# iamwinter/UMPR

Hardware: AMD Instinct MI355X
Metric: training samples/sec (higher is better)
Workload: dtype f32

## Files before the change

### include/umpr_hip.h

```cpp
#ifndef UMPR_HIP_H
#define UMPR_HIP_H
#include <stddef.h>
#include <stdint.h>

#ifdef __cplusplus
extern "C" {
#endif

const char* umpr_version(void);
const char* umpr_last_error(void);
int umpr_device_info(int dev, char* name, int name_len, int* compute_units, size_t* hbm_bytes);

int umpr_gemm_f32(const float* A, long lda, int transA, const float* B, long ldb, int transB, float* C, long ldc,
                  int M, int N, int K, const float* bias, int bias_mode, int act, int accumulate, float alpha,
                  float* ws, size_t ws_bytes, void* stream);

int umpr_set_gemm_bf16(int on);

int umpr_set_conv_inference(int on);

int umpr_set_conv_pool_follows(int on);

long umpr_debug_wino_fix_count(void);

int umpr_debug_conv3x3_plan(int pass, int N, int Cin, int Cout, int H, int W, int inference, size_t* ws_bytes, size_t* v_bytes);

int umpr_debug_wino_pool_fold(const float* y, const float* g_pooled, const float* w, const float* x, float* unpooled, float* dx,
                              float* dw, float* db, int N, int Cin, int Cout, int H, int W, int f4, int fold, float* ws,
                              size_t ws_bytes, void* stream);

size_t umpr_embed_gru_bidir_ws_bytes(int N, int L, int E);
int umpr_embed_gru_bidir_fwd(const int64_t* ids, const float* emb, int E,
                             const float* w_ih_f, const float* w_hh_f, const float* b_ih_f, const float* b_hh_f,
                             const float* w_ih_r, const float* w_hh_r, const float* b_ih_r, const float* b_hh_r,
                             const int32_t* lengths, const int32_t* order, const int32_t* dst_row, int N, int L,
                             float* out, float* saved, float* ws, size_t ws_bytes, void* stream);
int umpr_embed_gru_bidir_bwd(const int64_t* ids, const float* emb, int E,
                             const float* w_hh_f, const float* w_hh_r,
                             const int32_t* lengths, const int32_t* order, const int32_t* dst_row, int N, int L,
                             const float* dout, const float* out, const float* saved,
                             float* dw_ih_f, float* dw_hh_f, float* db_ih_f, float* db_hh_f,
                             float* dw_ih_r, float* dw_hh_r, float* db_ih_r, float* db_hh_r,
                             float* ws, size_t ws_bytes, void* stream);

int umpr_embed_gru_bidir_bwd_acc(const int64_t* ids, const float* emb, int E,
                                 const float* w_hh_f, const float* w_hh_r,
                                 const int32_t* lengths, const int32_t* order, const int32_t* dst_row, int N, int L,
                                 const float* dout, const float* out, const float* saved,
                                 float* dw_ih_f, float* dw_hh_f, float* db_ih_f, float* db_hh_f,
                                 float* dw_ih_r, float* dw_hh_r, float* db_ih_r, float* db_hh_r,
                                 int accumulate, float* ws, size_t ws_bytes, void* stream);

int umpr_embed_gru_bidir_bwd_dx(const int64_t* ids, const float* emb, int E,
                                const float* w_hh_f, const float* w_hh_r,
                                const int32_t* lengths, const int32_t* order, const int32_t* dst_row, int N, int L,
                                const float* dout, const float* out, const float* saved,
                                float* dw_ih_f, float* dw_hh_f, float* db_ih_f, float* db_hh_f,
                                float* dw_ih_r, float* dw_hh_r, float* db_ih_r, float* db_hh_r,
                                int accumulate, const float* w_ih_f, const float* w_ih_r, float* dx, int dx_accumulate,
                                float* ws, size_t ws_bytes, void* stream);

int umpr_embed_grad_chunk(void);
size_t umpr_embed_grad_ws_bytes(long T, int E);
int umpr_embed_grad(const int64_t* const* ids, const float* const* dx, const long* counts, int n_src, int E, long vocab,
                    const int32_t* sorted_pos, float* d_emb, void* ws, size_t ws_bytes, void* stream);

size_t umpr_embed_grad_rows_ws_bytes(long T, int E);
int umpr_embed_grad_rows(const int64_t* const* ids, const float* const* dx, const long* counts, int n_src, int E, long vocab,
                         const int32_t* sorted_pos, int64_t* row_id, float* row_grad, void* ws, size_t ws_bytes, void* stream);
int umpr_sparse_adam_rows(float* p, float* m, float* v, long vocab, int E, const int64_t* row_id, const float* row_grad, long T,
                          double lr, double beta1, double beta2, double eps, long step, double grad_scale,
                          const float* clip_state , void* stream);

size_t umpr_coattention_fwd_ws_bytes(int B, int SL);
int umpr_coattention_fwd(const float* Gu, const float* Gi, const float* M, int B, int SL, float* T, float* soft_u,
                         float* soft_i, float* atte_u, long ld_u, float* atte_i, long ld_i, float* colmax,
// ... 271 lines not shown
```

### umpr_amd/_lib.py

```python
from __future__ import annotations

import ctypes
import os
import threading

import torch

_HERE = os.path.dirname(os.path.abspath(__file__))
LIB_PATH = os.path.join(_HERE, "libumpr_hip.so")

_T = {"p": ctypes.c_void_p, "i": ctypes.c_int, "l": ctypes.c_long, "z": ctypes.c_size_t, "f": ctypes.c_float,
      "d": ctypes.c_double, "u": ctypes.c_uint64}

SIGNATURES = {
    "umpr_version": ("", "s"),
    "umpr_last_error": ("", "s"),
    "umpr_device_info": ("ipipp", "i"),
    "umpr_gemm_f32": ("pliplipliiipiiifpzp", "i"),
    "umpr_embed_gru_bidir_ws_bytes": ("iii", "z"),
    "umpr_embed_gru_bidir_fwd": ("ppipppppppppppiipppzp", "i"),
    "umpr_embed_gru_bidir_bwd": ("ppipppppiippppppppppppzp", "i"),
    "umpr_embed_gru_bidir_bwd_acc": ("ppipppppiipppppppppppipzp", "i"),
    "umpr_embed_gru_bidir_bwd_dx": ("ppipppppiipppppppppppipppipzp", "i"),
    "umpr_embed_grad_chunk": ("", "i"),
# ... 57 lines not shown
    "umpr_vgg16_bf16_act_bytes": ("i", "z"),
    "umpr_vgg16_bf16_fwd_ws_bytes": ("i", "z"),
    "umpr_vgg16_bf16_bwd_ws_bytes": ("i", "z"),
    "umpr_vgg16_bf16_features_fwd": ("ppipppzp", "i"),
    "umpr_vgg16_bf16_features_bwd": ("ppippppzp", "i"),
    "umpr_vgg16_cls_arena_bytes": ("i", "z"),
    "umpr_vgg16_classifier_fwd_compact": ("piiiuppppzp", "i"),
    "umpr_vgg16_classifier_bwd_compact": ("piippppppzp", "i"),
    "umpr_vgg16_classifier_fwd_compact_bf16": ("piiiuppppzp", "i"),
    "umpr_vgg16_classifier_bwd_compact_bf16": ("piippppppzp", "i"),
    "umpr_concat_ids": ("pplpp", "i"),
    "umpr_review_net_arena_bytes": ("iii", "z"),
    "umpr_review_net_ws_bytes": ("iiii", "z"),
    "umpr_review_net_fwd": ("ppipppiiiiiipppzp", "i"),
    "umpr_review_net_fwd_masked": ("ppipppiiiiiipppzpp", "i"),
    "umpr_review_net_bwd": ("ppipppiiiippppzp", "i"),
    "umpr_review_net_bwd_dx": ("ppipppiiiipppppzp", "i"),
    "umpr_review_net_fwd_ex": ("ppippppiiiiiipppzpp", "i"),
    "umpr_review_net_bwd_ex": ("ppippppiiiipppppzp", "i"),
    "umpr_control_net_arena_bytes": ("iiiiiii", "z"),
    "umpr_control_net_ws_bytes": ("iiiiiiiii", "z"),
    "umpr_control_net_fwd": ("pppipppppiiiiiiiifiippppppzp", "i"),
    "umpr_control_net_bwd": ("pppipppppiiiiiiiiipppppppzp", "i"),
    "umpr_control_net_bwd_dx": ("pppipppppiiiiiiiiipppppppppzp", "i"),
    "umpr_control_net_fwd_ex": ("pppipppppppiiiiiiiifiippppppzppp", "i"),
    "umpr_control_net_bwd_ex": ("pppipppppppiiiiiiiiipppppppppzp", "i"),
    "umpr_head_fwd": ("pppppppppppppfiiipppppppp", "i"),
    "umpr_head_bwd": ("pppppppppppfiiippppppppppppppppppppp", "i"),
    "umpr_photo_resize_u8": ("pzpiiipp", "i"),
    "umpr_photo_store_slot_bytes": ("ii", "z"),
    "umpr_photo_fetch_u8": ("pzpppiiiplpp", "i"),
    "umpr_photo_fetch_augment_u8": ("pzppppiiiplplpppp", "i"),
    "umpr_feature_fetch_f32": ("pipppiiplpp", "i"),
    "umpr_review_collate": ("pplppppppplpiiiiilpppp", "i"),
    "umpr_review_collate_sampled": ("pplppppppplpiiiiil" "iuil" "pppp", "i"),
    "umpr_bce_head_fwd": ("plpppiipppzp", "i"),
    "umpr_bce_head_bwd": ("plpppppiiplpppzp", "i"),
    "umpr_adam_step": ("ppppldddddldp", "i"),
    "umpr_sq_err_accumulate": ("pplpp", "i"),
    "umpr_adam_step_dev": ("pppplddd" "pp", "i"),
    "umpr_grad_norm_ws_bytes": ("", "z"),
    "umpr_grad_norm": ("ppidfppzpp", "i"),
    "umpr_adam_step_clip": ("ppppldddddld" "pp", "i"),
    "umpr_adam_step_dev_clip": ("pppplddd" "ppp", "i"),
    "umpr_adam_step_groups": ("ppppldddddld" "pp" "ppp" "ii" "p", "i"),
    "umpr_grad_accumulate": ("pppiip", "i"),
    "umpr_ema_update": ("pppidip", "i"),
    "umpr_arena_swap": ("pppip", "i"),
    "umpr_debug_poison_lds": ("pp", "i"),
    "umpr_set_gemm_bf16": ("i", "i"),
    "umpr_set_conv_inference": ("i", "i"),
    "umpr_set_conv_pool_follows": ("i", "i"),
    "umpr_debug_wino_fix_count": ("", "l"),
    "umpr_debug_conv3x3_plan": ("iiiiiiipp", "i"),
    "umpr_debug_wino_pool_fold": ("pppppppp" "iiiiiii" "pzp", "i"),
    "umpr_profile_enable": ("i", "i"),
    "umpr_profile_reset": ("", "i"),
    "umpr_profile_read": ("ippp", "i"),
}


class UmprHipError(RuntimeError):
    pass


class _Tls(threading.local):
    gemm_b16 = False


TLS = _Tls()


class _Lib:
    def __init__(self):
        if not os.path.exists(LIB_PATH):
            raise UmprHipError(
                f"{LIB_PATH} not found: build it with `python -c 'import __graft_entry__ as g; g.build()'` "
                f"(or `make -C umpr_amd/csrc`).  There is no CPU fallback.")
        self.cdll = ctypes.CDLL(LIB_PATH)
        self.fn = {}
        for name, (args, ret) in SIGNATURES.items():
            f = getattr(self.cdll, name)
            f.argtypes = [_T[c] for c in args]
            f.restype = {"i": ctypes.c_int, "z": ctypes.c_size_t, "s": ctypes.c_char_p, "p": ctypes.c_void_p,
                         "l": ctypes.c_long}[ret]
            self.fn[name] = f

    def last_error(self) -> str:
        return self.fn["umpr_last_error"]().decode()

    def call(self, name, *args):
        conv = []
        for a in args:
            if isinstance(a, torch.Tensor):
                conv.append(a.data_ptr())
            elif a is None:
                conv.append(None)
            else:
                conv.append(a)
        if TLS.gemm_b16:
            self.fn["umpr_set_gemm_bf16"](1)
            try:
                rc = self.fn[name](*conv)
            finally:
                self.fn["umpr_set_gemm_bf16"](0)
        else:
# ... 37 lines not shown
```

### umpr_amd/csrc/api.hip

```cpp
#include <math.h>
#include <stdarg.h>
#include <stdlib.h>

#include <vector>

#include "../../include/umpr_hip.h"
#include "umpr_common.h"
#include "umpr_internal.h"

static thread_local char g_err[512] = "";
void umpr_set_error(const char* fmt, ...) {
  va_list ap;
  va_start(ap, fmt);
  vsnprintf(g_err, sizeof(g_err), fmt, ap);
  va_end(ap);
}

namespace {
const bool g_fc_small = umpr_env_on("UMPR_FC_SMALL");
struct ProfRec { hipEvent_t e0, e1; int family; double work; };
bool g_prof_on = false;
std::vector<ProfRec> g_prof;
std::vector<ProfRec> g_prof_pool;
double g_prof_ms[UMPR_K_COUNT] = {0}, g_prof_work[UMPR_K_COUNT] = {0};
// ... 37 lines not shown
    for (int j = 0; j < kConvPerBlock[b]; ++j) {
      L.conv_cin[ci] = cin; L.conv_cout[ci] = kBlockCh[b]; L.conv_hw[ci] = hw; L.conv_block[ci] = b;
      L.conv_off[ci] = off;
      off += (size_t)n * kBlockCh[b] * hw * hw;
      cin = kBlockCh[b];
      ++ci;
    }
    hw /= 2;
    L.pool_off[b] = off;
    off += (size_t)n * kBlockCh[b] * hw * hw;
  }
  for (int j = 0; j < 2; ++j) { L.fc_off[j] = off; off += (size_t)n * 4096; }
  for (int j = 0; j < 2; ++j) { L.drop_off[j] = off; off += (size_t)n * 4096; }
  for (int i = 0; i < 13; ++i) {
    L.v_floats[i] = umpr_conv3x3_plan(CONV_FWD, n, L.conv_cin[i], L.conv_cout[i], L.conv_hw[i], L.conv_hw[i], false).v_floats;
    L.v_off[i] = off;
    off += L.v_floats[i];
  }
  L.total = off;
  return L;
}
}

extern "C" {

const char* umpr_version(void) { return "umpr_hip 0.1 (gfx950)"; }
const char* umpr_last_error(void) { return g_err; }

int umpr_device_info(int dev, char* name, int name_len, int* compute_units, size_t* hbm_bytes) {
  hipDeviceProp_t prop;
  if (hipGetDeviceProperties(&prop, dev) != hipSuccess) { umpr_set_error("device_info: no device %d", dev); return -1; }
  if (name && name_len > 0) { strncpy(name, prop.name, name_len - 1); name[name_len - 1] = 0; }
  if (compute_units) *compute_units = prop.multiProcessorCount;
  if (hbm_bytes) *hbm_bytes = prop.totalGlobalMem;
  return 0;
}

int umpr_gemm_f32(const float* A, long lda, int transA, const float* B, long ldb, int transB, float* C, long ldc,
                  int M, int N, int K, const float* bias, int bias_mode, int act, int accumulate, float alpha,
                  float* ws, size_t ws_bytes, void* stream) {
  UmprGemm g;
  g.A = A; g.lda = lda; g.transA = transA != 0; g.B = B; g.ldb = ldb; g.transB = transB != 0; g.C = C; g.ldc = ldc;
  g.M = M; g.N = N; g.K = K; g.bias = bias; g.bias_mode = bias_mode; g.act = act; g.accumulate = accumulate != 0;
  g.alpha = alpha; g.split_k = ws ? 0 : 1; g.ws = ws; g.ws_bytes = ws_bytes;
  return umpr_gemm(g, S(stream));
}

int umpr_set_gemm_bf16(int on) { umpr_gemm_set_b16(on != 0); return 0; }
static thread_local bool t_conv_inference = false, t_conv_pool_follows = false;
int umpr_set_conv_inference(int on) { t_conv_inference = on != 0; return 0; }
int umpr_set_conv_pool_follows(int on) { t_conv_pool_follows = on != 0; return 0; }
static ConvHints conv_hints() { ConvHints h; h.inference = t_conv_inference; h.pool_follows = t_conv_pool_follows; return h; }
long umpr_debug_wino_fix_count(void) { return umpr_wino_last_fix_count(); }
int umpr_debug_conv3x3_plan(int pass, int N, int Cin, int Cout, int H_, int W, int inference, size_t* ws_bytes, size_t* v_bytes) {
  UMPR_REQUIRE(pass >= CONV_FWD && pass <= CONV_WGRAD && N > 0 && Cin > 0 && Cout > 0 && H_ > 0 && W > 0, "conv3x3_plan: bad arguments");
  const ConvPlan p = umpr_conv3x3_plan(static_cast<ConvPass>(pass), N, Cin, Cout, H_, W, inference != 0);
  if (ws_bytes) *ws_bytes = p.ws_floats * sizeof(float);
  if (v_bytes) *v_bytes = p.v_floats * sizeof(float);
  return p.algo;
}
int umpr_debug_wino_pool_fold(const float* y, const float* g_pooled, const float* w, const float* x, float* unpooled, float* dx,
                              float* dw, float* db, int N, int Cin, int Cout, int H_, int W, int f4, int fold, float* ws,
                              size_t ws_bytes, void* stream) {
  UMPR_REQUIRE(N > 0 && Cin > 0 && Cout > 0 && H_ > 0 && W > 0 && (H_ % 2) == 0 && (W % 2) == 0 && y && g_pooled && ws,
               "debug_wino_pool_fold: bad arguments");
  UMPR_REQUIRE(fold || unpooled, "debug_wino_pool_fold: the un-folded run needs the buffer for the un-pooled gradient");
  UMPR_REQUIRE(!dx || (f4 && w), "debug_wino_pool_fold: the data gradient runs on the 4x4 tile and needs the weights");
  UMPR_REQUIRE(!dw || (x && (!f4 || ((H_ % 4) == 0 && (W % 4) == 0))), "debug_wino_pool_fold: the weight gradient on the 4x4 tile has no edge tiles");
  hipStream_t s = S(stream);
  ConvHints h;
  const float* g = g_pooled;
  if (fold) { h.pooled_dy = true; h.pool_y = y; }
  else {
    if (int rc = umpr_maxpool2_bwd_relu_impl(y, g_pooled, unpooled, (long)N * Cout, H_, W, s)) return rc;
    g = unpooled;
  }
  if (dx)
    if (int rc = umpr_wino_conv3x3(g, w, 1, nullptr, nullptr, dx, N, Cin, Cout, H_, W, 0, ws, ws_bytes / sizeof(float), true, h, s)) return rc;
  if (dw)
    if (int rc = umpr_wino_wgrad(g, x, dw, db, N, Cin, Cout, H_, W, 0, ws, ws_bytes / sizeof(float), f4 != 0, h, s)) return rc;
  return 0;
}

constexpr size_t kSlabs = 256;
namespace {
struct GruWs {
  float *gx, *wslab, *bslab;
  float* kslab; size_t kslab_bytes;
  float *stacked, *rows;
  float *wst, *bst;
  size_t bytes;
};
GruWs gru_ws(float* base, int N, int L, int pitch) {
  Carve c(base, sizeof(float));
  const size_t tiles = umpr_gru_tiles(N);
  GruWs w;
  w.gx = c.take<float>((size_t)N * L * 384); w.wslab = c.take<float>(tiles * 2 * G3 * H); w.bslab = c.take<float>(tiles * 2 * 2 * G3);
  w.wst = c.at<float>(c.off); w.bst = c.at<float>(c.off + (size_t)2 * G3 * pitch * sizeof(float));
  w.kslab_bytes = kSlabs * G3 * pitch * sizeof(float); w.kslab = c.take<float>(kSlabs * G3 * pitch);
  w.stacked = c.take<float>((size_t)2 * G3 * pitch); w.rows = c.take<float>((size_t)N * L * pitch); w.bytes = c.off;
  return w;
}
const bool g_emb_gather = umpr_env_on("UMPR_EMB_GATHER");
__global__ __launch_bounds__(256) void gather_rows_kernel(const int64_t* __restrict__ ids, const float* __restrict__ emb,
                                                          int E, int Ep, float* __restrict__ out, long rows) {
  const int lane = threadIdx.x & 63;
// ... 933 lines not shown
```

### umpr_amd/csrc/umpr_internal.h

```cpp
#pragma once
#include <hip/hip_runtime.h>
#include <stdint.h>

struct UmprGemm {
  const float* A = nullptr; long lda = 0; bool transA = false;
  const float* B = nullptr; long ldb = 0; bool transB = false;
  float* C = nullptr; long ldc = 0;
  int M = 0, N = 0, K = 0;
  const int64_t* gatherA = nullptr;
  const int64_t* gatherB = nullptr;
  const float* bias = nullptr; int bias_mode = 0;
  int act = 0; bool accumulate = false; float alpha = 1.0f;
  int split_k = 1;
  float* ws = nullptr; size_t ws_bytes = 0;
  int winA_L = 0, winA_D = 1, winA_pad = 0;
  int winB_L = 0, winB_D = 1, winB_pad = 0;
};
void umpr_gemm_set_b16(int on);
int umpr_gemm_b16();
int umpr_gemm(const UmprGemm& g, hipStream_t stream);
struct UmprB16Scope {
  int prev;
  explicit UmprB16Scope(int on) : prev(umpr_gemm_b16()) { if (on) umpr_gemm_set_b16(1); }
  ~UmprB16Scope() { umpr_gemm_set_b16(prev); }
// ... 25 lines not shown

int umpr_fill(float* p, long n, float v, hipStream_t s);
int umpr_multi_copy(const float* const* src, float* const* dst, const long* n, const int* accumulate, int nseg, hipStream_t s);
int umpr_multi_colsum_rows(const float* const* src, const int* rows, const long* cols, const long* row_stride, float* const* dst,
                           const int* accumulate, int nseg, hipStream_t s);
int umpr_copy_or_add(const float* src, float* dst, long n, int accumulate, hipStream_t s);

struct UmprHead {
  const float* rr;
  const float* c_u; const float* c_i; const float* pp; const float* pn;
  const float* vgg;
  const float* pos_v; const float* neg_v;
  const float* lw; const float* lb;
  const float* fw; const float* fb;
  const float* labels;
  float rate;
  int B, V, P, F;
  float* pred; float* loss;
  float* z;
  float* img_emb; float* pos_match; float* neg_match;
  float* posneg_emb;
  const float* d_loss;
  const float* d_pred;
  float* d_rr; float* d_cu; float* d_ci; float* d_pp; float* d_pn;
  float* d_vgg; float* d_pos_v; float* d_neg_v; float* d_lw; float* d_lb; float* d_fw; float* d_fb;
};
int umpr_head_launch(const UmprHead& p, int backward, hipStream_t s);

enum ConvPass { CONV_FWD = 0, CONV_DGRAD = 1, CONV_WGRAD = 2 };
enum ConvAlgo { CONV_GENERIC = 0 , CONV_C3 = 1 ,
                CONV_DIRECT = 2 , CONV_WINO2 = 3, CONV_WINO4 = 4 };
struct ConvHints {
  bool inference = false, pool_follows = false; float* v_slot = nullptr; size_t v_slot_floats = 0;
  bool pooled_dy = false; const float* pool_y = nullptr;
};
struct ConvPlan {
  ConvAlgo algo;
  ConvAlgo direct;
  bool edge;
  size_t ws_floats;
  size_t v_floats;
};
ConvPlan umpr_conv3x3_plan(ConvPass pass, int N, int Cin, int Cout, int H, int W, bool inference);
size_t umpr_conv3x3_pack_floats(int N, int Cin, int Cout, int H, int W);
bool umpr_conv3x3_pool_fold_ok(int N, int Cin, int Cout, int H, int W);
int umpr_conv3x3_run(const float* x, const float* w, int transposed, const float* bias, const float* mask, float* y,
                     int N, int Cin, int Cout, int H, int W, int relu, float* wpack, size_t wpack_floats,
                     const ConvHints& hints, hipStream_t s);
struct WinoConvGeom { int planes, MT, S; long T, Tpad; bool edge; size_t v_floats, U, V, M, count, tie, floats; };
WinoConvGeom umpr_wino_conv_geom(int N, int C, int M, int H, int W, bool f4);
struct WinoWgradGeom { long T, Tpad; int MT, CT, Mpad, Cpad, stages, splits, stages_per_split, planes, bnc; size_t Gy, V, P, BP, floats; };
WinoWgradGeom umpr_wino_wgrad_geom(int N, int Cin, int Cout, int H, int W, bool f4);
long umpr_wino_last_fix_count();
int umpr_wino_wgrad(const float* dy, const float* x, float* dw, float* db, int N, int Cin, int Cout, int H, int W,
                    int accumulate, float* ws, size_t ws_floats, bool f4, const ConvHints& hints, hipStream_t s);
int umpr_wino_conv3x3(const float* x, const float* w, int transposed, const float* bias, const float* mask, float* y,
                      int N, int Cin, int Cout, int H, int W, int relu, float* ws, size_t ws_floats, bool f4,
                      const ConvHints& hints, hipStream_t s);
int umpr_conv3x3_flip_transpose(const float* w, float* wt, int Cout, int Cin, hipStream_t s);
size_t umpr_conv3x3_wgrad_ws_bytes(int N, int Cin, int Cout, int H, int W);
int umpr_conv3x3_wgrad(const float* gz, const float* x, float* dw, float* db, int N, int Cin, int Cout, int H, int W,
                       int accumulate, float* ws, size_t ws_bytes, const ConvHints& hints, hipStream_t s);
int umpr_maxpool2_fwd_impl(const float* x, float* y, long planes, int H, int W, hipStream_t s);
int umpr_maxpool2_bwd_relu_impl(const float* x, const float* gy, float* gx, long planes, int H, int W, hipStream_t s);

int umpr_wgrad_reduce(const float* slab, const float* bslab, int splits, int Cout, int Cin, float* dw, float* db,
                      int accumulate, hipStream_t s);

struct UmprPF {
  int N, H, W, RW;
  long rows;
  long ptot;
  long lead, tail;
  long ps;
};
UmprPF umpr_pf(int N, int H, int W);
size_t umpr_pf_bytes(const UmprPF& g, int C);
size_t umpr_conv_bf16_pack_bytes(int Cin, int Cout);
int umpr_conv_bf16_run(const void* x, const float* w, int transposed, const float* bias, const void* mask, void* y,
                       const UmprPF& g, int Cin, int Cout, int relu, void* wpack, size_t wpack_bytes, hipStream_t s,
                       bool zero_guards = true);
int umpr_conv_bf16_pack_all(const float* const* w, const int* Cin, const int* Cout, const int* W, int n, int transposed,
                            void* wpack, const size_t* offsets, hipStream_t s);
int umpr_pf_zero_guards_multi(void* const* bases, const UmprPF* geos, const int* channels, int n, hipStream_t s);
size_t umpr_wgrad_bf16_ws_bytes(const UmprPF& g, int Cin, int Cout);
int umpr_wgrad_bf16_run(const void* dy, const void* x, float* dw, float* db, const UmprPF& g, int Cin, int Cout,
                        int accumulate, float* ws, size_t ws_bytes, hipStream_t s);
int umpr_conv1_bf16_fwd(const float* x, const float* w, const float* bias, void* y, const UmprPF& g, hipStream_t s,
                        bool zero_guards = true);
size_t umpr_conv1_bf16_wgrad_ws_bytes();
int umpr_conv1_bf16_wgrad(const void* dy, const float* x, float* dw, float* db, const UmprPF& g, int accumulate, float* ws,
                          size_t ws_bytes, hipStream_t s);
int umpr_nchw_to_cb8(const float* x, void* y, const UmprPF& g, int C, hipStream_t s);
int umpr_cb8_to_nchw(const void* x, float* y, const UmprPF& g, int C, hipStream_t s);
int umpr_maxpool2_bf16_fwd_run(const void* x, void* y, const UmprPF& gi, const UmprPF& go, int C, hipStream_t s,
                               bool zero_guards = true);
int umpr_maxpool2_bf16_bwd_run(const void* x, const void* gy, void* gx, const UmprPF& gi, const UmprPF& go, int C,
                               hipStream_t s);

int umpr_colsum_rows(const float* src, int rows, long cols, long row_stride, float* dst, int accumulate, hipStream_t s);
int umpr_gru_recurrent_fwd(const float* gx, const float* whh_f, const float* bhh_f, const float* whh_r,
                           const float* bhh_r, const int* lengths, const int* order, const int* dst_row, float* out,
                           float* saved, int N, int L, hipStream_t s);
int umpr_gru_tiles(int N);
int umpr_gru_bptt(const float* dout, const float* out, const float* saved, const float* whh_f, const float* whh_r,
                  const int* lengths, const int* order, const int* dst_row, float* dgx, float* dwhh_slab,
// ... 69 lines not shown
```

### umpr_amd/csrc/winograd.hip

```cpp
#include <type_traits>

#include "umpr_common.h"
#include "umpr_internal.h"

namespace {

constexpr int WK = 32;
constexpr int WBM = 128;
constexpr int WBN = 128;

__device__ __forceinline__ void pool_window_grad(const float2 a, const float2 b, const float gy, float2& ga, float2& gb) {
  int arg = 0;
  float m = a.x;
  if (a.y > m) { m = a.y; arg = 1; }
  if (b.x > m) { m = b.x; arg = 2; }
  if (b.y > m) { m = b.y; arg = 3; }
  const float g = m > 0.f ? gy : 0.f;
  ga = make_float2(arg == 0 ? g : 0.f, arg == 1 ? g : 0.f);
  gb = make_float2(arg == 2 ? g : 0.f, arg == 3 ? g : 0.f);
}
typedef float f32x4_t __attribute__((ext_vector_type(4)));
__device__ __forceinline__ float as_loaded(float v) { asm volatile("" : "+v"(v)); return v; }
__device__ __forceinline__ float4 as_loaded(const float4 v) {
  f32x4_t q = {v.x, v.y, v.z, v.w};
  asm volatile("" : "+v"(q));
  return make_float4(q.x, q.y, q.z, q.w);
}

__global__ void wino_weights_kernel(const float* __restrict__ w, float* __restrict__ U, int M, int C, int CinW,
                                    int transposed) {
  const int MT = (M + WBM - 1) / WBM, S = (C + WK - 1) / WK;
  const long total = (long)MT * WBM * S * WK;
  for (long i = blockIdx.x * (long)blockDim.x + threadIdx.x; i < total; i += (long)gridDim.x * blockDim.x) {
    const int ml = (int)(i % WBM);
    long r = i / WBM;
    const int k = (int)(r % WK); r /= WK;
    const int s = (int)(r % S);
    const int mt = (int)(r / S);
    const int m = mt * WBM + ml, c = s * WK + k;
    float g[9];
#pragma unroll
    for (int t = 0; t < 9; ++t) {
      float v = 0.f;
      if (m < M && c < C) v = transposed ? w[((long)c * CinW + m) * 9 + 8 - t] : w[((long)m * CinW + c) * 9 + t];
      g[t] = v;
    }
    float gg[4][3];
#pragma unroll
    for (int j = 0; j < 3; ++j) {
      gg[0][j] = g[j];
      gg[1][j] = 0.5f * (g[j] + g[3 + j] + g[6 + j]);
      gg[2][j] = 0.5f * (g[j] - g[3 + j] + g[6 + j]);
// ... 598 lines not shown
                                                         const unsigned int* __restrict__ list, const unsigned int* __restrict__ count,
                                                         unsigned cap, int C, int Mch, int H, int W, int relu) {
  const unsigned n_fix = min(*count, cap);
  const int lane = threadIdx.x & 63;
  const unsigned wave = blockIdx.x * 4 + (threadIdx.x >> 6), waves = gridDim.x * 4;
  const long HW = (long)H * W;
  for (unsigned i = wave; i < n_fix; i += waves) {
    const unsigned idx = list[i];
    const int xx = (int)(idx % W);
    unsigned r = idx / W;
    const int yy = (int)(r % H); r /= H;
    const int m = (int)(r % Mch);
    const int n = (int)(r / Mch);
    float acc = 0.f;
    for (int c = lane; c < C; c += 64) {
      const float* xp = x + ((long)n * C + c) * HW;
      const float* wp = w + ((long)m * C + c) * 9;
#pragma unroll
      for (int dy = 0; dy < 3; ++dy) {
        const int py = yy + dy - 1;
        if (py < 0 || py >= H) continue;
#pragma unroll
        for (int dx = 0; dx < 3; ++dx) {
          const int px = xx + dx - 1;
          if (px < 0 || px >= W) continue;
          acc = fmaf(xp[(long)py * W + px], wp[dy * 3 + dx], acc);
        }
      }
    }
#pragma unroll
    for (int o = 32; o > 0; o >>= 1) acc += __shfl_xor(acc, o, 64);
    if (lane == 0) {
      float v = acc + (bias ? bias[m] : 0.f);
      if (relu) v = fmaxf(v, 0.f);
      y[idx] = v;
    }
  }
}

static long wino_tpad(long T) { return (T + WBN - 1) / WBN * WBN; }

struct WinoGemmParams {
  const float* U;
  const float* V;
  float* Mx;
  int MT, S, C;
  long Tpad;
  long TT;
  int Mpad;
  int planes;
};

typedef __attribute__((address_space(3))) void* lds_ptr_t;
template <int FOLD>
__global__ __launch_bounds__(256, 2) void wino_gemm_dma_kernel(WinoGemmParams p) {
  constexpr int SK = WK;
  constexpr int LD = 128;
  constexpr int TM = 2, TN = 2;
  constexpr int KS = SK / 2;
  constexpr int NP = SK / 8;
  constexpr int SFLUSH = 1;
  typedef typename std::conditional<FOLD == 2, double, float>::type tot_t;
  __shared__ __attribute__((aligned(1024))) float As[2][SK * LD];
  __shared__ __attribute__((aligned(1024))) float Bs[2][SK * LD];
  const int tid = threadIdx.x, lane = tid & 63;
  const int wave = __builtin_amdgcn_readfirstlane(tid >> 6);
  const int wm = wave >> 1, wn = wave & 1;
  const int l31 = lane & 31, half = lane >> 5;
  const long TT = p.TT;
  const int xcd = blockIdx.x & 7;
  const long qq = blockIdx.x >> 3;
  const int mt = (int)(qq % p.MT);
  const long bt = (qq / p.MT) * 8 + xcd;
  if (bt >= p.planes * TT) return;
  const int xi = (int)(bt / TT);
  const long t0 = (bt % TT) * WBN;
  const float* Ub = p.U + (((long)xi * p.MT + mt) * p.S) * (WK * WBM);
  const float* Vb = p.V + (long)xi * (p.S * WK) * p.Tpad + t0;
  const float* ga = Ub + wave * (NP * 256) + lane * 4;
  const float* gb = Vb + (long)(wave * (2 * NP) + half) * p.Tpad + l31 * 4;
  const long bstep = 2 * p.Tpad;
  const unsigned lds_a = (unsigned)(size_t)(lds_ptr_t)(&As[0][0]) + (unsigned)wave * (NP * 1024u);
  const unsigned lds_b = (unsigned)(size_t)(lds_ptr_t)(&Bs[0][0]) + (unsigned)wave * (NP * 1024u);
  auto glds = [&](const float* src, unsigned dst) {
    unsigned keep;
    asm volatile("s_mov_b32 %0, m0\n\ts_mov_b32 m0, %2\n\ts_nop 0\n\tglobal_load_lds_dwordx4 %1, off\n\ts_mov_b32 m0, %0"
                 : "=&s"(keep) : "v"(src), "s"(dst) : "memory");
  };
  auto dma = [&](int q, int sn, int nbuf) {
    if (q < NP) glds(ga + (long)sn * (SK * WBM) + q * 256, lds_a + (unsigned)nbuf * (SK * LD * 4u) + (unsigned)q * 1024u);
    else glds(gb + (long)sn * SK * p.Tpad + (q - NP) * bstep, lds_b + (unsigned)nbuf * (SK * LD * 4u) + (unsigned)(q - NP) * 1024u);
  };
  auto dma_wait = [&]() { asm volatile("s_waitcnt vmcnt(0)" ::: "memory"); };

  f32x16 acc[TM][TN];
  tot_t tot[TM][TN][16];
#pragma unroll
  for (int i = 0; i < TM; ++i)
#pragma unroll
    for (int j = 0; j < TN; ++j)
#pragma unroll
      for (int r = 0; r < 16; ++r) { acc[i][j][r] = 0.f; tot[i][j][r] = (tot_t)0; }

  const int ns = p.S * (WK / SK);
#pragma unroll
  for (int q = 0; q < 2 * NP; ++q) dma(q, 0, 0);
  dma_wait();
  __syncthreads();
  for (int s0 = 0; s0 < ns; s0 += SFLUSH) {
#pragma unroll
    for (int i = 0; i < TM; ++i)
#pragma unroll
      for (int j = 0; j < TN; ++j)
#pragma unroll
        for (int r = 0; r < 16; ++r) acc[i][j][r] = 0.f;
    const int s1 = min(ns, s0 + SFLUSH);
    for (int s = s0; s < s1; ++s) {
      const int cur = s & 1;
      const int sn = min(s + 1, ns - 1);
      const float* as = As[cur] + half * LD + wm * 64 + l31;
      const float* bs = Bs[cur] + half * LD + wn * 64 + l31;
      float a[2][TM], b[2][TN];
#pragma unroll
      for (int i = 0; i < TM; ++i) a[0][i] = as[i * 32];
#pragma unroll
      for (int j = 0; j < TN; ++j) b[0][j] = bs[j * 32];
#pragma unroll
      for (int kk = 0; kk < KS; ++kk) {
        const int cb = kk & 1, nb = cb ^ 1;
        const int k1 = kk + 1;
#pragma unroll
        for (int m = 0; m < TM * TN; ++m) {
          const int i = m / TN, j = m % TN;
          acc[i][j] = mfma32(a[cb][i], b[cb][j], acc[i][j]);
          if (m == 0 && k1 < KS) {
#pragma unroll
            for (int ii = 0; ii < TM; ++ii) a[nb][ii] = as[2 * k1 * LD + ii * 32];
          }
          if (m == 1 && k1 < KS) {
#pragma unroll
            for (int jj = 0; jj < TN; ++jj) b[nb][jj] = bs[2 * k1 * LD + jj * 32];
          }
          if (m == 3 && kk < 2 * NP) dma(kk, sn, cur ^ 1);
          __builtin_amdgcn_sched_barrier(0);
        }
      }
      dma_wait();
      __syncthreads();
    }
#pragma unroll
    for (int i = 0; i < TM; ++i)
#pragma unroll
      for (int j = 0; j < TN; ++j)
#pragma unroll
        for (int r = 0; r < 16; ++r) tot[i][j][r] += (tot_t)acc[i][j][r];
  }
  float* Mb = p.Mx + ((long)xi * p.Mpad + mt * WBM) * p.Tpad + t0;
#pragma unroll
  for (int i = 0; i < TM; ++i)
#pragma unroll
    for (int j = 0; j < TN; ++j)
#pragma unroll
      for (int r = 0; r < 16; ++r)
        Mb[(long)(wm * 64 + i * 32 + mfma_row(r, lane)) * p.Tpad + wn * 64 + j * 32 + l31] = (float)tot[i][j][r];
}

inline int nblk(long n, int cap) {
  long b = (n + 255) / 256;
  if (b > cap) b = cap;
  return (int)(b < 1 ? 1 : b);
}

}

static thread_local const unsigned int* t_last_fix_count = nullptr;
long umpr_wino_last_fix_count() {
  if (!t_last_fix_count) return -1;
  unsigned int v = 0;
  if (hipDeviceSynchronize() != hipSuccess || hipMemcpy(&v, t_last_fix_count, sizeof(v), hipMemcpyDeviceToHost) != hipSuccess) return -2;
  return (long)v;
}

WinoConvGeom umpr_wino_conv_geom(int N, int C, int M, int H, int W, bool f4) {
  WinoConvGeom g;
  g.planes = f4 ? 36 : 16; g.edge = f4 && ((H % 4) != 0 || (W % 4) != 0);
  g.T = f4 ? (long)N * ((H + 3) / 4) * ((W + 3) / 4) : (long)N * (H / 2) * (W / 2);
  g.Tpad = wino_tpad(g.T); g.MT = (M + WBM - 1) / WBM; g.S = (C + WK - 1) / WK;
  g.v_floats = (size_t)g.planes * g.S * WK * g.Tpad;
  g.U = 0; g.V = (size_t)g.planes * g.MT * WBM * g.S * WK; g.M = g.V + g.v_floats;
  g.count = g.M + (size_t)g.planes * g.MT * WBM * g.Tpad; g.tie = g.count + 16;
  g.floats = g.count + 64 + (f4 ? g.Tpad : 0);
  return g;
}


int umpr_wino_conv3x3(const float* x, const float* w, int transposed, const float* bias, const float* mask, float* y,
                      int N, int Cin, int Cout, int H, int W, int relu, float* ws, size_t ws_floats, bool f4,
                      const ConvHints& hints, hipStream_t s) {
  const int M = transposed ? Cin : Cout;
  const int C = transposed ? Cout : Cin;
  const WinoConvGeom G = umpr_wino_conv_geom(N, C, M, H, W, f4);
  UMPR_REQUIRE(ws_floats >= G.floats, "winograd: workspace too small");
  UMPR_REQUIRE((H % 2) == 0 && (W % 2) == 0, "winograd: odd map %dx%d", H, W);
  const int planes = G.planes, MT = G.MT, S = G.S;
  const long T = G.T, Tpad = G.Tpad; const bool edge = G.edge;
  float *U = ws + G.U, *V = ws + G.V, *Mx = ws + G.M, *list_region = ws + G.V;
  if (hints.v_slot) {
    UMPR_REQUIRE(f4 && !edge && !transposed && hints.v_slot_floats == G.v_floats,
                 "winograd: the V slot does not fit this forward (%d -> %d at %dx%d)", Cin, Cout, H, W);
    V = hints.v_slot;
  }
  if (f4) wino4_weights_kernel<<<nblk((long)MT * WBM * S * WK, 2048), 256, 0, s>>>(w, U, M, C, Cin, transposed, wino4_consts());
  else wino_weights_kernel<<<nblk((long)MT * WBM * S * WK, 2048), 256, 0, s>>>(w, U, M, C, Cin, transposed);
  UMPR_LAUNCH_CHECK("wino_weights");
  const long TT = (T + WBN - 1) / WBN;
  static const int kappa = umpr_env_int("UMPR_WINO_FIX_KAPPA", 8);
  const bool fix = f4 && !transposed && !hints.inference && kappa > 0 && mask == nullptr;
  WinoFix fx{nullptr, nullptr, 0u, 0.f, nullptr};
  unsigned int* tie_bits = nullptr;
  if (fix) {
    fx.count = reinterpret_cast<unsigned int*>(ws + G.count);
    fx.list = reinterpret_cast<unsigned int*>(list_region);
    fx.cap = (unsigned)(G.v_floats < (size_t)0x7fffffff ? G.v_floats : (size_t)0x7fffffff);
    fx.kappa_eps = (float)kappa * 5.9604644775390625e-08f;
    UMPR_REQUIRE((long)N * M * H * W < 0xffffffffL, "winograd fix-up: output tensor too large for 32-bit element indices");
    if (hints.pool_follows) {
      tie_bits = reinterpret_cast<unsigned int*>(ws + G.tie);
      if (hipMemsetAsync(tie_bits - 1, 0, (size_t)(T + 1) * sizeof(unsigned int), s) != hipSuccess) { umpr_set_error("winograd fix-up: memset"); return -2; }
      UMPR_REQUIRE(((long)N * C * H * W) % 4 == 0 && (reinterpret_cast<uintptr_t>(x) & 15) == 0, "winograd fix-up: unaligned input");
      wino_absmax_kernel<<<nblk((long)N * C * H * W / 4, 1024), 256, 0, s>>>(x, (long)N * C * H * W / 4, tie_bits - 1);
      UMPR_LAUNCH_CHECK("wino_absmax");
      fx.tie_bits = tie_bits;
    }
  }
  if (hints.pooled_dy) {
    UMPR_REQUIRE(f4 && transposed && hints.pool_y && !fix, "winograd: the pooled source needs a data gradient on the 4x4 tile");
    if (edge) wino4_input_kernel<true, false, true><<<nblk((long)S * WK * TT * WBN, 16384), 256, 0, s>>>(x, V, N, C, S * WK, H, W, Tpad, TT * WBN, wino4_consts(), nullptr, nullptr, hints.pool_y);
    else wino4_input_kernel<false, false, true><<<nblk((long)S * WK * TT * WBN, 16384), 256, 0, s>>>(x, V, N, C, S * WK, H, W, Tpad, TT * WBN, wino4_consts(), nullptr, nullptr, hints.pool_y);
  } else if (f4 && edge) {
    if (tie_bits) wino4_input_kernel<true, true><<<nblk((long)S * WK * TT * WBN, 16384), 256, 0, s>>>(x, V, N, C, S * WK, H, W, Tpad, TT * WBN, wino4_consts(), fx.count, tie_bits);
    else wino4_input_kernel<true, false><<<nblk((long)S * WK * TT * WBN, 16384), 256, 0, s>>>(x, V, N, C, S * WK, H, W, Tpad, TT * WBN, wino4_consts(), fx.count, nullptr);
  } else if (f4) {
    if (tie_bits) wino4_input_kernel<false, true><<<nblk((long)S * WK * TT * WBN, 16384), 256, 0, s>>>(x, V, N, C, S * WK, H, W, Tpad, TT * WBN, wino4_consts(), fx.count, tie_bits);
    else wino4_input_kernel<false, false><<<nblk((long)S * WK * TT * WBN, 16384), 256, 0, s>>>(x, V, N, C, S * WK, H, W, Tpad, TT * WBN, wino4_consts(), fx.count, nullptr);
  }
  else if ((W / 2) % 2 == 0)
    wino_input_pair_kernel<<<nblk((long)S * WK * TT * WBN / 2, 16384), 256, 0, s>>>(x, V, N, C, S * WK, H, W, Tpad, TT * WBN);
  else
    wino_input_kernel<<<nblk((long)S * WK * TT * WBN, 16384), 256, 0, s>>>(x, V, N, C, S * WK, H, W, Tpad, TT * WBN);
  UMPR_LAUNCH_CHECK("wino_input");
  WinoGemmParams p{U, V, Mx, MT, S, C, Tpad, TT, MT * WBM, planes};
  const long groups = (planes * TT + 7) / 8 * 8;
  {
    UmprProfScope prof(UMPR_K_WINO_GEMM, 2.0 * planes * (double)M * C * T, s);
    static const int fold = umpr_env_int("UMPR_WINO_FOLD", 1);
    if (fold == 2) wino_gemm_dma_kernel<2><<<(unsigned)(groups * MT), 256, 0, s>>>(p);
    else wino_gemm_dma_kernel<1><<<(unsigned)(groups * MT), 256, 0, s>>>(p);
  }
  UMPR_LAUNCH_CHECK("wino_gemm");
  if (f4 && fix) {
    if (edge) wino4_output_kernel<true, true><<<nblk((long)M * T, 16384), 256, 0, s>>>(Mx, bias, mask, y, N, M, H, W, Tpad, MT * WBM, relu, wino4_consts(), fx);
    else wino4_output_kernel<false, true><<<nblk((long)M * T, 16384), 256, 0, s>>>(Mx, bias, mask, y, N, M, H, W, Tpad, MT * WBM, relu, wino4_consts(), fx);
    UMPR_LAUNCH_CHECK("wino_output");
    wino_fixup_kernel<<<128, 256, 0, s>>>(x, w, bias, y, fx.list, fx.count, fx.cap, C, M, H, W, relu);
    UMPR_LAUNCH_CHECK("wino_fixup");
    t_last_fix_count = fx.count;
    return 0;
  }
  if (f4 && edge)
    wino4_output_kernel<true, false><<<nblk((long)M * T, 16384), 256, 0, s>>>(Mx, bias, mask, y, N, M, H, W, Tpad, MT * WBM, relu, wino4_consts(), fx);
  else if (f4)
    wino4_output_kernel<false, false><<<nblk((long)M * T, 16384), 256, 0, s>>>(Mx, bias, mask, y, N, M, H, W, Tpad, MT * WBM, relu, wino4_consts(), fx);
  else if ((W / 2) % 2 == 0)
    wino_output_pair_kernel<<<nblk((long)M * T / 2, 16384), 256, 0, s>>>(Mx, bias, mask, y, N, M, H, W, Tpad, MT * WBM, relu);
  else
    wino_output_kernel<<<nblk((long)M * T, 16384), 256, 0, s>>>(Mx, bias, mask, y, N, M, H, W, Tpad, MT * WBM, relu);
  UMPR_LAUNCH_CHECK("wino_output");
  return 0;
}

namespace {

template <bool POOL>
__global__ void wino_dy_kernel(const float* __restrict__ dy, float* __restrict__ Gy, int N, int Mch, int H, int W,
                               long Tpad, long Tw, int Mpad, const float* __restrict__ pool_y) {
  const int TH = H / 2, TW = W / 2;
  const long T = (long)N * TH * TW;
  const long total = (long)Mch * Tw;
  const long per = (long)Mpad * Tpad;
  for (long i = blockIdx.x * (long)blockDim.x + threadIdx.x; i < total; i += (long)gridDim.x * blockDim.x) {
    const long t = i % Tw;
    const int m = (int)(i / Tw);
    float* dst = Gy + (long)m * Tpad + t;
    if (t >= T) {
#pragma unroll
      for (int a = 0; a < 16; ++a) dst[(long)a * per] = 0.f;
      continue;
    }
    const int tx = (int)(t % TW);
    const long r = t / TW;
    const int ty = (int)(r % TH), n = (int)(r / TH);
    const long o = (((long)n * Mch + m) * H + 2 * ty) * W + 2 * tx;
    float2 g0, g1;
    if (POOL) {
      pool_window_grad(*reinterpret_cast<const float2*>(pool_y + o), *reinterpret_cast<const float2*>(pool_y + o + W),
                       dy[((long)n * Mch + m) * TH * TW + (long)ty * TW + tx], g0, g1);
    } else {
      g0 = *reinterpret_cast<const float2*>(dy + o);
      g1 = *reinterpret_cast<const float2*>(dy + o + W);
    }
// ... 573 lines not shown
```

Measured before the change: 2184.

## Add 64-column Winograd GEMM tile variant chosen by a wave-quantization cost model

Templates the Winograd batched GEMM kernel on its column tile width, adding a 64-wide variant with smaller LDS footprint and three workgroups per CU. A host-side cost model compares rounds of workgroups across the device's CUs for both widths and picks 64 when the 128 grid would leave a partially filled final wave. This targets tail-wave underutilization on layers whose block count does not divide evenly across CUs, at the cost of less B-tile reuse per workgroup and a heuristic constant that may mispredict. A debug override and a query API are also exposed.

```diff
diff --git a/include/umpr_hip.h b/include/umpr_hip.h
--- a/include/umpr_hip.h
+++ b/include/umpr_hip.h
@@ -22,6 +22,10 @@
 int umpr_set_conv_pool_follows(int on);
 
 long umpr_debug_wino_fix_count(void);
+
+int umpr_wino_gemm_width(int planes, long T, int MT, int S, int cus, double* cost128, double* cost64);
+
+int umpr_debug_set_wino_gemm_width(int width);
 
 int umpr_debug_conv3x3_plan(int pass, int N, int Cin, int Cout, int H, int W, int inference, size_t* ws_bytes, size_t* v_bytes);
 
diff --git a/umpr_amd/_lib.py b/umpr_amd/_lib.py
--- a/umpr_amd/_lib.py
+++ b/umpr_amd/_lib.py
@@ -133,6 +133,8 @@
     "umpr_set_conv_inference": ("i", "i"),
     "umpr_set_conv_pool_follows": ("i", "i"),
     "umpr_debug_wino_fix_count": ("", "l"),
+    "umpr_wino_gemm_width": ("iliiipp", "i"),
+    "umpr_debug_set_wino_gemm_width": ("i", "i"),
     "umpr_debug_conv3x3_plan": ("iiiiiiipp", "i"),
     "umpr_debug_wino_pool_fold": ("pppppppp" "iiiiiii" "pzp", "i"),
     "umpr_profile_enable": ("i", "i"),
diff --git a/umpr_amd/csrc/api.hip b/umpr_amd/csrc/api.hip
--- a/umpr_amd/csrc/api.hip
+++ b/umpr_amd/csrc/api.hip
@@ -113,6 +113,10 @@
 int umpr_set_conv_pool_follows(int on) { t_conv_pool_follows = on != 0; return 0; }
 static ConvHints conv_hints() { ConvHints h; h.inference = t_conv_inference; h.pool_follows = t_conv_pool_follows; return h; }
 long umpr_debug_wino_fix_count(void) { return umpr_wino_last_fix_count(); }
+int umpr_wino_gemm_width(int planes, long T, int MT, int S, int cus, double* cost128, double* cost64) {
+  return umpr_wino_gemm_pick(planes, T, MT, S, cus, cost128, cost64);
+}
+int umpr_debug_set_wino_gemm_width(int width) { return umpr_wino_force_gemm_width(width); }
 int umpr_debug_conv3x3_plan(int pass, int N, int Cin, int Cout, int H_, int W, int inference, size_t* ws_bytes, size_t* v_bytes) {
   UMPR_REQUIRE(pass >= CONV_FWD && pass <= CONV_WGRAD && N > 0 && Cin > 0 && Cout > 0 && H_ > 0 && W > 0, "conv3x3_plan: bad arguments");
   const ConvPlan p = umpr_conv3x3_plan(static_cast<ConvPass>(pass), N, Cin, Cout, H_, W, inference != 0);
diff --git a/umpr_amd/csrc/umpr_internal.h b/umpr_amd/csrc/umpr_internal.h
--- a/umpr_amd/csrc/umpr_internal.h
+++ b/umpr_amd/csrc/umpr_internal.h
@@ -101,6 +101,8 @@
 struct WinoWgradGeom { long T, Tpad; int MT, CT, Mpad, Cpad, stages, splits, stages_per_split, planes, bnc; size_t Gy, V, P, BP, floats; };
 WinoWgradGeom umpr_wino_wgrad_geom(int N, int Cin, int Cout, int H, int W, bool f4);
 long umpr_wino_last_fix_count();
+int umpr_wino_gemm_pick(int planes, long T, int MT, int S, int cus, double* cost128, double* cost64);
+int umpr_wino_force_gemm_width(int width);
 int umpr_wino_wgrad(const float* dy, const float* x, float* dw, float* db, int N, int Cin, int Cout, int H, int W,
                     int accumulate, float* ws, size_t ws_floats, bool f4, const ConvHints& hints, hipStream_t s);
 int umpr_wino_conv3x3(const float* x, const float* w, int transposed, const float* bias, const float* mask, float* y,
diff --git a/umpr_amd/csrc/winograd.hip b/umpr_amd/csrc/winograd.hip
--- a/umpr_amd/csrc/winograd.hip
+++ b/umpr_amd/csrc/winograd.hip
@@ -1,3 +1,4 @@
+#include <atomic>
 #include <type_traits>
 
 #include "umpr_common.h"
@@ -702,17 +703,21 @@
 };
 
 typedef __attribute__((address_space(3))) void* lds_ptr_t;
-template <int FOLD>
-__global__ __launch_bounds__(256, 2) void wino_gemm_dma_kernel(WinoGemmParams p) {
+template <int FOLD, int BN>
+__global__ __launch_bounds__(256, BN == 64 ? 3 : 2) void wino_gemm_dma_kernel(WinoGemmParams p) {
+  static_assert(BN == 128 || BN == 64, "tile columns per workgroup");
   constexpr int SK = WK;
   constexpr int LD = 128;
-  constexpr int TM = 2, TN = 2;
+  constexpr int TM = 2, TN = BN / 64;
   constexpr int KS = SK / 2;
   constexpr int NP = SK / 8;
+  constexpr int NPB = SK * BN / 1024;
+  constexpr int LPR = BN / 4;
+  constexpr int RPP = 64 / LPR;
   constexpr int SFLUSH = 1;
   typedef typename std::conditional<FOLD == 2, double, float>::type tot_t;
   __shared__ __attribute__((aligned(1024))) float As[2][SK * LD];
-  __shared__ __attribute__((aligned(1024))) float Bs[2][SK * LD];
+  __shared__ __attribute__((aligned(1024))) float Bs[2][SK * BN];
   const int tid = threadIdx.x, lane = tid & 63;
   const int wave = __builtin_amdgcn_readfirstlane(tid >> 6);
   const int wm = wave >> 1, wn = wave & 1;
@@ -724,14 +729,15 @@
   const long bt = (qq / p.MT) * 8 + xcd;
   if (bt >= p.planes * TT) return;
   const int xi = (int)(bt / TT);
-  const long t0 = (bt % TT) * WBN;
+  const long t0 = (bt % TT) * BN;
   const float* Ub = p.U + (((long)xi * p.MT + mt) * p.S) * (WK * WBM);
   const float* Vb = p.V + (long)xi * (p.S * WK) * p.Tpad + t0;
   const float* ga = Ub + wave * (NP * 256) + lane * 4;
-  const float* gb = Vb + (long)(wave * (2 * NP) + half) * p.Tpad + l31 * 4;
-  const long bstep = 2 * p.Tpad;
+  const int brow = BN == 128 ? half : lane / LPR, bcol = BN == 128 ? l31 : lane % LPR;
+  const float* gb = Vb + (long)(wave * (RPP * NPB) + brow) * p.Tpad + bcol * 4;
+  const long bstep = RPP * p.Tpad;
   const unsigned lds_a = (unsigned)(size_t)(lds_ptr_t)(&As[0][0]) + (unsigned)wave * (NP * 1024u);
-  const unsigned lds_b = (unsigned)(size_t)(lds_ptr_t)(&Bs[0][0]) + (unsigned)wave * (NP * 1024u);
+  const unsigned lds_b = (unsigned)(size_t)(lds_ptr_t)(&Bs[0][0]) + (unsigned)wave * (NPB * 1024u);
   auto glds = [&](const float* src, unsigned dst) {
     unsigned keep;
     asm volatile("s_mov_b32 %0, m0\n\ts_mov_b32 m0, %2\n\ts_nop 0\n\tglobal_load_lds_dwordx4 %1, off\n\ts_mov_b32 m0, %0"
@@ -739,7 +745,7 @@
   };
   auto dma = [&](int q, int sn, int nbuf) {
     if (q < NP) glds(ga + (long)sn * (SK * WBM) + q * 256, lds_a + (unsigned)nbuf * (SK * LD * 4u) + (unsigned)q * 1024u);
-    else glds(gb + (long)sn * SK * p.Tpad + (q - NP) * bstep, lds_b + (unsigned)nbuf * (SK * LD * 4u) + (unsigned)(q - NP) * 1024u);
+    else glds(gb + (long)sn * SK * p.Tpad + (q - NP) * bstep, lds_b + (unsigned)nbuf * (SK * BN * 4u) + (unsigned)(q - NP) * 1024u);
   };
   auto dma_wait = [&]() { asm volatile("s_waitcnt vmcnt(0)" ::: "memory"); };
 
@@ -754,7 +760,7 @@
 
   const int ns = p.S * (WK / SK);
 #pragma unroll
-  for (int q = 0; q < 2 * NP; ++q) dma(q, 0, 0);
+  for (int q = 0; q < NP + NPB; ++q) dma(q, 0, 0);
   dma_wait();
   __syncthreads();
   for (int s0 = 0; s0 < ns; s0 += SFLUSH) {
@@ -769,7 +775,7 @@
       const int cur = s & 1;
       const int sn = min(s + 1, ns - 1);
       const float* as = As[cur] + half * LD + wm * 64 + l31;
-      const float* bs = Bs[cur] + half * LD + wn * 64 + l31;
+      const float* bs = Bs[cur] + half * BN + wn * (BN / 2) + l31;
       float a[2][TM], b[2][TN];
 #pragma unroll
       for (int i = 0; i < TM; ++i) a[0][i] = as[i * 32];
@@ -789,9 +795,9 @@
           }
           if (m == 1 && k1 < KS) {
 #pragma unroll
-            for (int jj = 0; jj < TN; ++jj) b[nb][jj] = bs[2 * k1 * LD + jj * 32];
+            for (int jj = 0; jj < TN; ++jj) b[nb][jj] = bs[2 * k1 * BN + jj * 32];
           }
-          if (m == 3 && kk < 2 * NP) dma(kk, sn, cur ^ 1);
+          if (m == TM * TN - 1 && kk < NP + NPB) dma(kk, sn, cur ^ 1);
           __builtin_amdgcn_sched_barrier(0);
         }
       }
@@ -812,7 +818,7 @@
     for (int j = 0; j < TN; ++j)
 #pragma unroll
       for (int r = 0; r < 16; ++r)
-        Mb[(long)(wm * 64 + i * 32 + mfma_row(r, lane)) * p.Tpad + wn * 64 + j * 32 + l31] = (float)tot[i][j][r];
+        Mb[(long)(wm * 64 + i * 32 + mfma_row(r, lane)) * p.Tpad + wn * (BN / 2) + j * 32 + l31] = (float)tot[i][j][r];
 }
 
 inline int nblk(long n, int cap) {
@@ -829,6 +835,38 @@
   unsigned int v = 0;
   if (hipDeviceSynchronize() != hipSuccess || hipMemcpy(&v, t_last_fix_count, sizeof(v), hipMemcpyDeviceToHost) != hipSuccess) return -2;
   return (long)v;
+}
+
+constexpr int kWinoGemm128PerCu = 2, kWinoGemm64PerCu = 3;
+constexpr double kWinoGemm64Cost = 1.04;
+static double wino_gemm_rounds_cost(long blocks, int bn, int S, int cus) {
+  const int per_cu = bn == 64 ? kWinoGemm64PerCu : kWinoGemm128PerCu;
+  const long slots = (long)per_cu * cus;
+  return (double)((blocks + slots - 1) / slots) * ((double)S * 16.0 * (bn / 32)) * per_cu * (bn == 64 ? kWinoGemm64Cost : 1.0);
+}
+static int wino_device_cus() {
+  static const int cus = [] {
+    int dev = 0, n = 0;
+    if (hipGetDevice(&dev) != hipSuccess || hipDeviceGetAttribute(&n, hipDeviceAttributeMultiprocessorCount, dev) != hipSuccess) n = 0;
+    return n;
+  }();
+  return cus;
+}
+int umpr_wino_gemm_pick(int planes, long T, int MT, int S, int cus, double* cost128, double* cost64) {
+  UMPR_REQUIRE(planes > 0 && T > 0 && MT > 0 && S > 0, "wino_gemm_width: bad arguments");
+  if (cus <= 0) cus = wino_device_cus();
+  UMPR_REQUIRE(cus > 0, "wino_gemm_width: no device to take the CU count from");
+  const long b128 = (long)planes * ((T + 127) / 128) * MT, b64 = (long)planes * ((T + 63) / 64) * MT;
+  const double c128 = wino_gemm_rounds_cost(b128, 128, S, cus), c64 = wino_gemm_rounds_cost(b64, 64, S, cus);
+  if (cost128) *cost128 = c128;
+  if (cost64) *cost64 = c64;
+  return b128 > (long)kWinoGemm128PerCu * cus && c64 < c128 ? 64 : 128;
+}
+static std::atomic<int> g_wino_gemm_width{0};
+int umpr_wino_force_gemm_width(int width) {
+  UMPR_REQUIRE(width == 0 || width == 64 || width == 128, "debug_set_wino_gemm_width: %d is not 0, 64 or 128", width);
+  g_wino_gemm_width.store(width);
+  return 0;
 }
 
 WinoConvGeom umpr_wino_conv_geom(int N, int C, int M, int H, int W, bool f4) {
@@ -899,13 +937,19 @@
   else
     wino_input_kernel<<<nblk((long)S * WK * TT * WBN, 16384), 256, 0, s>>>(x, V, N, C, S * WK, H, W, Tpad, TT * WBN);
   UMPR_LAUNCH_CHECK("wino_input");
-  WinoGemmParams p{U, V, Mx, MT, S, C, Tpad, TT, MT * WBM, planes};
-  const long groups = (planes * TT + 7) / 8 * 8;
+  int bn = g_wino_gemm_width.load();
+  if (bn == 0) bn = umpr_wino_gemm_pick(planes, T, MT, S, 0, nullptr, nullptr);
+  if (bn < 0) return bn;
+  const long TTg = (T + bn - 1) / bn;
+  WinoGemmParams p{U, V, Mx, MT, S, C, Tpad, TTg, MT * WBM, planes};
+  const long groups = (planes * TTg + 7) / 8 * 8;
   {
     UmprProfScope prof(UMPR_K_WINO_GEMM, 2.0 * planes * (double)M * C * T, s);
     static const int fold = umpr_env_int("UMPR_WINO_FOLD", 1);
-    if (fold == 2) wino_gemm_dma_kernel<2><<<(unsigned)(groups * MT), 256, 0, s>>>(p);
-    else wino_gemm_dma_kernel<1><<<(unsigned)(groups * MT), 256, 0, s>>>(p);
+    if (fold == 2 && bn == 64) wino_gemm_dma_kernel<2, 64><<<(unsigned)(groups * MT), 256, 0, s>>>(p);
+    else if (fold == 2) wino_gemm_dma_kernel<2, 128><<<(unsigned)(groups * MT), 256, 0, s>>>(p);
+    else if (bn == 64) wino_gemm_dma_kernel<1, 64><<<(unsigned)(groups * MT), 256, 0, s>>>(p);
+    else wino_gemm_dma_kernel<1, 128><<<(unsigned)(groups * MT), 256, 0, s>>>(p);
   }
   UMPR_LAUNCH_CHECK("wino_gemm");
   if (f4 && fix) {
```

After: 2188 (median of 2 runs). About the same (+0.2%).
